# MariusDoe/fractal-ray-marching

Hardware: AMD Instinct MI355X
Metric: Gray-march-steps/sec + frames/sec, 4K Mandelbulb 12-iter/256-step, 1 & 8 GPU (higher is better)
Workload: dtype f32

## Files before the change

### fractal-ray-marching_amd/csrc/frm_render_kernels.h

```cpp
#pragma once
#include "frm_internal.h"
#include "frm_srgb_table.h"

namespace frm {

__device__ __forceinline__ unsigned long long wave_sum(unsigned long long v) {
#pragma unroll
  for (int off = 32; off >= 1; off >>= 1) v += __shfl_xor(v, off, 64);
  return v;
}

__device__ __forceinline__ uint32_t band_row_to_global(const BandGeometry& g, uint32_t lr) {
  uint32_t b = lr / g.band_rows;
  return (g.first_band + b * g.band_stride) * g.band_rows + (lr - b * g.band_rows);
}

template <uint32_t FAM, bool ITERS>
__global__ __launch_bounds__(256) void render_simple(KernelArgs a) {
  __shared__ float table[256];
  table[threadIdx.x] = kSrgbThresholds[threadIdx.x];
  __syncthreads();

  const uint32_t wave = threadIdx.x >> 6, lane = threadIdx.x & 63u;
  const uint32_t x = blockIdx.x * 16u + (wave & 1u) * 8u + (lane & 7u);
  const uint32_t lr = blockIdx.y * 16u + (wave >> 1) * 8u + (lane >> 3);
  const uint32_t width = a.f.width;

  uint32_t n_pix = 0;
  PixelCount pc = {0u, 0u, 0u, 0u, {0u, 0u}};
  if (x < width && lr < a.g.local_rows) {
    const uint32_t y = band_row_to_global(a.g, lr);
    if (y < a.f.height) {
      n_pix = 1;
      v3 color = shade_pixel<FAM, ITERS>(a.f, a.s, x, y, pc);
      a.out[(size_t)lr * width + x] = pack_rgba(color, table);
    }
  }

  unsigned long long v[7] = {n_pix, pc.hit, pc.primary, pc.shadow, pc.normal, pc.de.bodies, pc.de.bailouts};
#pragma unroll
  for (int k = 0; k < 7; ++k) {
    unsigned long long s = wave_sum(v[k]);
    if (lane == 0 && s) atomicAdd(&a.counters[k], s);
  }
}

constexpr uint32_t kIdle = 0xFFFFFFFFu;
constexpr uint32_t kChunk = 64u;


enum Phase : uint32_t { kPrimary = 0, kTap0 = 1, kTap3 = 4, kShadow = 5 };

__device__ __forceinline__ uint32_t uniform(uint32_t v) { return __builtin_amdgcn_readfirstlane(v); }
__device__ __forceinline__ uint32_t queue_part() {
  const uint32_t xcc = __builtin_amdgcn_s_getreg((3 << 11) | 20) & (kXcds - 1u);
  constexpr uint32_t per = kQueueParts / kXcds;
  return xcc * per + (per > 1u ? (blockIdx.x / kXcds) % per : 0u);
}
__device__ __forceinline__ uint64_t count(bool c) { return (uint64_t)__popcll(ballot(c)); }

__device__ __forceinline__ uint8_t cost_key(uint32_t bodies) {
  return (uint8_t)min(255.0f, 16.0f * __log2f((float)bodies + 1.0f));
}

__device__ __forceinline__ uint32_t sys_load(const uint32_t* p) {
  return __hip_atomic_load(p, __ATOMIC_RELAXED, __HIP_MEMORY_SCOPE_SYSTEM);
}
__device__ __forceinline__ void sys_store(uint32_t* p, uint32_t v) {
  __hip_atomic_store(p, v, __ATOMIC_RELAXED, __HIP_MEMORY_SCOPE_SYSTEM);
}
template <class T>
__device__ __forceinline__ T dev_poll(T* p) {
  return __hip_atomic_fetch_add(p, (T)0, __ATOMIC_RELAXED, __HIP_MEMORY_SCOPE_AGENT);
}
template <class T>
__device__ __forceinline__ T dev_load(const T* p) {
  return __hip_atomic_load(p, __ATOMIC_RELAXED, __HIP_MEMORY_SCOPE_AGENT);
}
template <class T>
__device__ __forceinline__ void dev_store(T* p, T v) {
  __hip_atomic_store(p, v, __ATOMIC_RELAXED, __HIP_MEMORY_SCOPE_AGENT);
}
__device__ __forceinline__ void ring_wait_mem() { asm volatile("s_waitcnt vmcnt(0)" ::: "memory"); }
__device__ __forceinline__ uint64_t realtime() { return __builtin_amdgcn_s_memrealtime(); }
constexpr uint64_t kRingWatchdogTicks = 200000000ull;
constexpr unsigned long long kEpochMask = 0xFFFFFFFF00000000ull;
__device__ __forceinline__ unsigned long long epoch_of(uint32_t seq) { return (unsigned long long)seq << 32; }
#ifdef FRM_RING_TRACE
#define RING_TRACE_MIN(r, seq, k) atomicMin(&(r).dev->trace[(seq) & 63u][k], (unsigned long long)realtime())
#define RING_TRACE_MAX(r, seq, k) atomicMax(&(r).dev->trace[(seq) & 63u][k], (unsigned long long)realtime())
#define RING_GRID_TRACE(r, k) atomicMin(&(r).dev->grid_trace[(r).grid_id & 63u][k], (unsigned long long)realtime())
#else
#define RING_TRACE_MIN(r, seq, k)
#define RING_TRACE_MAX(r, seq, k)
#define RING_GRID_TRACE(r, k)
#endif
__device__ __forceinline__ RingFrameCtl& ring_ctl(const RingArgs& r, uint32_t seq) {
  return r.dev->set[(seq - 1u) & (2u * r.slots - 1u)];
}
struct RingLds {
  RingHost* host;
  RingDev* dev;
  uint32_t* order;
  uint32_t slots, grid_id, rec_stride, npix;
};
__device__ __forceinline__ uint32_t rl_u32(const volatile uint32_t& v) { return uniform(v); }
template <class T>
__device__ __forceinline__ T* rl_ptr(T* const volatile& v) {
  const uint64_t x = reinterpret_cast<uint64_t>(v);
  return reinterpret_cast<T*>((uint64_t)uniform((uint32_t)x) | ((uint64_t)uniform((uint32_t)(x >> 32)) << 32));
}
__device__ __forceinline__ RingArgs ring_view(const volatile RingLds* rl) {
  RingArgs r;
  r.host = rl_ptr(rl->host);
  r.dev = rl_ptr(rl->dev);
  r.order = rl_ptr(rl->order);
  r.slots = rl_u32(rl->slots);
  r.grid_id = rl_u32(rl->grid_id);
  r.first_seq = 0;
  r.service_waves = 0;
  r.out = nullptr;
  r.keys = nullptr;
  return r;
}

__device__ __forceinline__ uint32_t epoch_add(unsigned long long* w, uint32_t seq, uint32_t v) {
  unsigned long long old = 0;
  if ((threadIdx.x & 63u) == 0) old = atomicAdd(w, (unsigned long long)v);
  old = __shfl(old, 0, 64);
  return (old & kEpochMask) == epoch_of(seq) ? (uint32_t)old : 0xFFFFFFFFu;
}
__device__ __forceinline__ uint32_t epoch_claim(unsigned long long* w, uint32_t seq, uint32_t n) {
  const uint32_t t = epoch_add(w, seq, 1u);
  return t < n ? t : 0xFFFFFFFFu;
}

struct RingView {
  uint32_t limit;
  bool closed;
};
__device__ __forceinline__ void ring_refresh(const RingArgs& r, RingView& v) {
  if (v.closed) return;
  uint32_t lim = 0, closed = 0;
  if ((threadIdx.x & 63u) == 0) {
    closed = dev_poll(&r.dev->grid.limit_valid);
    if (closed) {
      lim = dev_poll(&r.dev->grid.limit);
    } else {
      const uint32_t posted = sys_load(&r.host->posted);
      const uint32_t stop = sys_load(&r.host->grid_stop[r.grid_id % kRingGridIds][0]);
      lim = min(posted, stop - 1u);
#ifdef FRM_RING_TRACE
      if (lim >= 1u) RING_TRACE_MIN(r, lim, 0);
#endif
    }
  }
  v.closed = uniform(__shfl(closed, 0, 64)) != 0;
  v.limit = uniform(__shfl(lim, 0, 64));
}
__device__ __forceinline__ void ring_close(const RingArgs& r, RingView& v) {
  uint32_t lim = 0, ok = 1;
  if ((threadIdx.x & 63u) == 0) {
    if (atomicCAS(&r.dev->grid.closed, 0u, 1u) == 0u) {
      sys_store(&r.host->closed, r.grid_id);
      RING_GRID_TRACE(r, 1);
      ring_wait_mem();
      const uint32_t posted = sys_load(&r.host->posted);
      const uint32_t stop = sys_load(&r.host->grid_stop[r.grid_id % kRingGridIds][0]);
      lim = min(posted, stop - 1u);
      atomicExch(&r.dev->grid.limit, lim);
      atomicExch(&r.dev->base, lim + 1u);
      ring_wait_mem();
      atomicExch(&r.dev->grid.limit_valid, 1u);
    } else {
      const uint64_t t0 = realtime();
      while (!dev_poll(&r.dev->grid.limit_valid)) {
        if (realtime() - t0 > 1000000ull) { ok = 0; break; }
        __builtin_amdgcn_s_sleep(2);
      }
      lim = dev_poll(&r.dev->grid.limit);
    }
  }
  v.closed = true;
  v.limit = uniform(__shfl(ok ? lim : 0u, 0, 64));
}

struct RingCam {
  float row[3][4];
  v3 origin;
  float power;
  uint32_t* host_img;
};
__device__ __forceinline__ void ring_camera_lds(const RingArgs& r, uint32_t slot, float* lds) {
  const uint32_t* w = reinterpret_cast<const uint32_t*>(&r.host->frames[slot]);
  const uint32_t lane = threadIdx.x & 63u;
  if (lane < 16u) lds[lane] = __uint_as_float(sys_load(w + lane));
  __syncthreads();
}
__device__ __forceinline__ RingCam ring_camera(const RingArgs& r, uint32_t slot) {
  const uint32_t* w = reinterpret_cast<const uint32_t*>(&r.host->frames[slot]);
  const uint32_t lane = threadIdx.x & 63u;
  const uint32_t mine = lane < 20u ? sys_load(w + lane) : 0u;
  RingCam c;
#pragma unroll
  for (int i = 0; i < 12; ++i) c.row[i / 4][i % 4] = __uint_as_float(uniform(__shfl(mine, i, 64)));
  c.origin = mk(__uint_as_float(uniform(__shfl(mine, 12, 64))), __uint_as_float(uniform(__shfl(mine, 13, 64))),
                __uint_as_float(uniform(__shfl(mine, 14, 64))));
  c.power = __uint_as_float(uniform(__shfl(mine, 15, 64)));
  const uint64_t lo = uniform(__shfl(mine, 18, 64)), hi = uniform(__shfl(mine, 19, 64));
  c.host_img = reinterpret_cast<uint32_t*>(lo | (hi << 32));
  return c;
}
// ... 233 lines not shown
    const uint32_t pos = atomicAdd(&cnt[dev_load(&keys[idx])], 1u);
    if (pos < npix) dev_store(&order[pos], idx);
  }
}

__device__ __forceinline__ void ring_finish(const KernelArgs& a, uint32_t seq, uint32_t s) {
  const uint32_t lane = threadIdx.x & 63u;
  const uint32_t next_seq = seq + a.ring.slots;
  RingFrameCtl& c = ring_ctl(a.ring, next_seq);
  const unsigned long long next = epoch_of(next_seq);
  if (lane <= kQueueParts) dev_store(&c.queue[lane * (kQueuePartWords / 2u)], next);
  if (lane == 16u) dev_store(&c.pix_done[0], next);
  if (lane == 17u) dev_store(&c.shade_next[0], next);
  if (lane == 18u) dev_store(&c.shade_done[0], next);
  if (lane == 19u) dev_store(&c.rank_next[0], next);
  if (lane == 20u) dev_store(&c.rank_done[0], next);
#pragma unroll
  for (uint32_t k = 0; k < kRankWords / 64u; ++k) dev_store(&c.hist[k * 64u + lane], 0u);
  __builtin_amdgcn_fence(__ATOMIC_RELEASE, "");
  if (lane == 0) {
    RING_TRACE_MIN(a.ring, seq, 5);
    atomicExch(&a.ring.dev->done_seq[s][0], seq);
    sys_store(&a.ring.host->done[s][0], seq);
  }
}

__device__ __forceinline__ void ring_idle() {
#pragma unroll
  for (int i = 0; i < 4; ++i) __builtin_amdgcn_s_sleep(127);
}

template <uint32_t FAM>
__device__ __noinline__ void ring_service(const KernelArgs& a, uint32_t* cnt) {
  const RingArgs& R = a.ring;
  const uint32_t lane = threadIdx.x & 63u;
  const float* table = kSrgbThresholds;
  const uint32_t npix = a.npix;
  const uint32_t ntask = (npix + kRingTaskPixels - 1u) / kRingTaskPixels;
  uint32_t seq0 = 0;
  if (lane == 0) seq0 = max(R.first_seq, dev_poll(&R.dev->base));
  seq0 = uniform(__shfl(seq0, 0, 64));
  RingView rv = {0u, false};
  uint64_t last_progress = realtime();
  unsigned long long last_pd = 0;
  for (;;) {
    if (seq0 > rv.limit) ring_refresh(R, rv);
    for (;;) {
      if (seq0 > rv.limit) break;
      uint32_t d = 0;
      if (lane == 0) d = dev_poll(&R.dev->done_seq[(seq0 - 1u) & (R.slots - 1u)][0]);
      if (uniform(__shfl(d, 0, 64)) < seq0) break;
      ++seq0;
    }
    if (seq0 > rv.limit) {
      if (rv.closed) return;
      if (realtime() - last_progress > kRingWatchdogTicks) return;
      ring_idle();
      continue;
    }
    bool worked = false;
    for (uint32_t g = seq0; g <= rv.limit && g < seq0 + R.slots && !worked; ++g) {
      const uint32_t s = (g - 1u) & (R.slots - 1u);
      RingFrameCtl& c = ring_ctl(R, g);
      unsigned long long pd = 0, sd = 0;
      if (lane == 0) {
        pd = dev_poll(&c.pix_done[0]);
        sd = dev_poll(&c.shade_done[0]);
      }
      pd = __shfl(pd, 0, 64);
      sd = __shfl(sd, 0, 64);
      if (g == seq0 && pd != last_pd) {
        last_pd = pd;
        last_progress = realtime();
      }
      if (pd != (epoch_of(g) | npix)) continue;
      if (sd == (epoch_of(g) | ntask)) {
        const uint32_t t = epoch_claim(&c.rank_next[0], g, ntask);
        if (t == kIdle) continue;
        ring_rank_task(a, g, s, t, cnt);
        ring_wait_mem();
        if (epoch_add(&c.rank_done[0], g, 1u) == ntask - 1u) ring_finish(a, g, s);
        worked = true;
      } else {
        const uint32_t t = epoch_claim(&c.shade_next[0], g, ntask);
        if (t == kIdle) continue;
        const RingCam cam = ring_camera(R, s);
        ring_shade_task<FAM>(a, cam, g, s, t, table, cnt);
        if (cam.host_img)
          __builtin_amdgcn_fence(__ATOMIC_RELEASE, "");
        else
          ring_wait_mem();
        if (epoch_add(&c.shade_done[0], g, 1u) == ntask - 1u && lane == 0) RING_TRACE_MIN(R, g, 4);
        worked = true;
      }
    }
    if (worked) {
      last_progress = realtime();
    } else {
      if (realtime() - last_progress > kRingWatchdogTicks) return;
      ring_idle();
    }
  }
}

#ifdef FRM_STAMPS
constexpr uint32_t kWaveDebugSlots = 16384u;
__device__ unsigned long long g_wave_debug[16u * kWaveDebugSlots];
#endif

template <uint32_t FAM, bool ITERS, bool MULTI = false, bool ANIM = false, bool RES = false>
#ifndef FRM_MARCH_WAVES_PER_SIMD
#define FRM_MARCH_WAVES_PER_SIMD 1
#endif
#ifndef FRM_RING_WAVES_PER_SIMD
#define FRM_RING_WAVES_PER_SIMD FRM_MARCH_WAVES_PER_SIMD
#endif
__global__ __launch_bounds__(kMarchBlock, RES ? FRM_RING_WAVES_PER_SIMD : FRM_MARCH_WAVES_PER_SIMD) void march_persistent(
    KernelArgs a) {
  __shared__ float4 chunk_rays[kMarchWaves][kChunk];
  static_assert(!RES || (!MULTI && kMarchWaves == 1u), "ring grids: one-wave workgroups, one frame per chunk");
  __shared__ float cam_lds[RES ? kRingSlots : 1][16];
  __shared__ uint32_t rw[RES ? (uint32_t)kRwWords : 1u];
  __shared__ RingLds ring_lds[RES ? 1 : 0 + 1];
  if constexpr (RES) {
    if (blockIdx.x < a.ring.service_waves) {
      ring_service<FAM>(*(const KernelArgs*)__builtin_amdgcn_kernarg_segment_ptr(),
                        reinterpret_cast<uint32_t*>(&chunk_rays[0][0]));
      return;
    }
  }

  const FrameUniforms& f = a.f;
  const SceneUniforms& su = a.s;
  constexpr bool kMb = is_mandelbulb(FAM);
  constexpr bool kHw = FAM == kMandelbulbHw;
  const uint32_t wave = threadIdx.x >> 6, lane = threadIdx.x & 63u;
  const uint64_t lane_bit = 1ull << lane;
  constexpr bool multi = MULTI;
  const uint32_t total = multi ? a.batch * ((a.npix + kChunk - 1u) / kChunk) * kChunk : a.npix;
  uint32_t chunk_frame = 0;
  const uint32_t n_iter = iterations<ITERS>(su.n);
  static_assert(!ANIM || ((MULTI || RES) && is_mandelbulb(FAM)), "per-lane powers: multi-frame or ring Mandelbulb launches");
  float lane_power = su.mb_power;
  ShadeGeom* __restrict__ geom = a.geom;
  ShadeTail* __restrict__ tails = a.tails;

  uint32_t slots_used = kChunk;
  bool exhausted = false;
  const uint32_t nchunks = (total + kChunk - 1u) / kChunk;
  uint32_t part = queue_part();
  uint64_t drained = 0;
  const uint32_t nhead = nchunks / kQueueHeadDiv;
  uint64_t n_pix = 0, n_hit = 0, n_prim = 0, n_shadow = 0, n_body = 0, n_bail = 0;
#ifdef FRM_COUNT_EXACT
  uint64_t n_dbg_total = 0, n_dbg_exact = 0;
#endif
  uint32_t r_slot = 0;
  if constexpr (RES) {
    uint32_t b = 0;
    if (lane == 0) {
      RING_GRID_TRACE(a.ring, 0);
      b = max(a.ring.first_seq, dev_poll(&a.ring.dev->base));
      ring_lds->host = a.ring.host;
      ring_lds->dev = a.ring.dev;
      ring_lds->order = a.ring.order;
      ring_lds->slots = a.ring.slots;
      ring_lds->grid_id = a.ring.grid_id;
      ring_lds->rec_stride = a.rec_stride;
      ring_lds->npix = a.npix;
    }
    __syncthreads();
    if (lane < (uint32_t)kRwWords) rw[lane] = 0u;
    rw_set(rw, kRwLo, uniform(__shfl(b, 0, 64)));
  }

  uint32_t pix = kIdle;
  uint32_t phase = kPrimary;
  bool done = false;
  v3 o = mk(0.f, 0.f, 0.f), d = o, nsum = o, q = o, z = o;
  float t = 0.f, closeness = 0.f, dr = 1.f, mag = 0.f, de = 0.f;
  uint32_t it = 0, psteps = 0, body = 0;
  uint32_t pix_cost = 0;
#ifdef FRM_STAMPS
  uint64_t stamp_service = 0, n_service = 0, n_loop = 0, real_exhaust = 0;
  uint64_t stamp_consume = 0, stamp_refill = 0, n_fetch = 0;
  uint64_t stamp_sub[4] = {0, 0, 0, 0};
  const uint64_t stamp_begin = __builtin_amdgcn_s_memtime();
  const uint64_t stamp_real0 = __builtin_amdgcn_s_memrealtime();
#define FRM_SUB_BEGIN() const uint64_t sub0 = __builtin_amdgcn_s_memtime()
#define FRM_SUB_END(k) stamp_sub[k] += __builtin_amdgcn_s_memtime() - sub0
#else
#define FRM_SUB_BEGIN()
#define FRM_SUB_END(k)
#endif

  for (;;) {
    if constexpr (kMb) {
      const uint64_t live = ballot(pix != kIdle);
      uint64_t pending = live & ~ballot(done);
      const uint64_t waitable = exhausted ? live : ~0ull;
      for (;;) {
        if (pending == 0 || (uint32_t)__popcll(waitable & ~pending) >= a.service_min) break;
        if constexpr (!RES) n_body += (uint64_t)__popcll(pending);
#ifdef FRM_STAMPS
        n_loop++;
#endif
        if (lane_in(pending)) {
#if defined(FRM_COUNT_EXACT) && defined(__HIP_DEVICE_COMPILE__)
          n_dbg_total++;
          if (ballot(!mb_tame(z, mag)) != 0) n_dbg_exact++;
#endif
          if constexpr (ANIM)
            mb_step<kHw>(lane_power, lane_power - 1.0f, q, mag, z, dr);
          else
            mb_step<kHw>(su, q, mag, z, dr);
          body++;
          if (body <= n_iter) mag = mb_length<kHw>(z);
        }
        pending &= ~(ballot(body > n_iter) | ballot(mag > su.mb_bailout));
      }
      done = !lane_in(pending);
    }

#ifdef FRM_STAMPS
    const uint64_t stamp0 = __builtin_amdgcn_s_memtime();
#endif
    const bool cons = pix != kIdle && done;
    bool ev_bail = false;
    bool plain_log = true;
    if constexpr (kMb && !kHw)
      plain_log = ballot(cons && !__builtin_amdgcn_classf(mag, 0x100 )) == 0;
    if (cons) {
      done = false;
      if constexpr (kMb) {
        FRM_SUB_BEGIN();
#if defined(__HIP_DEVICE_COMPILE__)
        if constexpr (kHw)
          de = mb_distance_hw(mag, dr);
        else
          de = plain_log ? mb_distance_posnormal(mag, dr) : mb_distance(mag, dr);
#else
        (void)plain_log;
        de = mb_distance(mag, dr);
#endif
        pix_cost += body;
        ev_bail = body <= n_iter;
        FRM_SUB_END(0);
      }
    }
    const bool ev_prim = cons && phase == kPrimary, ev_shadow = cons && phase == kShadow;
    const bool tap = cons && !ev_prim && !ev_shadow;
    const bool hit = de <= kMinDistance;
    const bool ev_hit = ev_prim && hit;
    const float cl = min_(closeness, de / t);
    closeness = ev_shadow ? cl : closeness;
    const bool step = (ev_prim || ev_shadow) && !hit;
    const float t_next = t + de;
    const uint32_t it_next = it + 1u;
    const bool more = it_next < f.max_steps && t_next < kMaxTotalDistance;
    t = step ? t_next : t;
    it = step ? it_next : it;
    psteps = ev_hit ? it : psteps;
    const bool fin = (step && !more) || (ev_shadow && hit);
    const bool sun_miss = ev_shadow && step && !more;
    bool need_point = ev_hit || (step && more) || tap;
    const uint32_t k = phase - kTap0;
    const float dx = (k == 0u || k == 3u) ? de : -de, dy = (k >= 2u) ? de : -de,
                dz = (k == 1u || k == 3u) ? de : -de;
    const float sx = (k == 0u) ? dx : nsum.x + dx, sy = (k == 0u) ? dy : nsum.y + dy,
                sz = (k == 0u) ? dz : nsum.z + dz;
    nsum = mk(tap ? sx : nsum.x, tap ? sy : nsum.y, tap ? sz : nsum.z);
    phase = ev_hit ? kTap0 : (tap ? phase + 1u : phase);
    if (tap && k == kTap3 - kTap0) {
      FRM_SUB_BEGIN();
#if defined(__HIP_DEVICE_COMPILE__)
      const v3 n = normalize_wave(nsum);
#else
      const v3 n = normalize(nsum);
#endif
      const v3 hp = ray_at(o, t, d);
      if constexpr (RES) {
        coherent_store(&geom[pix], make_float4(t, n.x, n.y, n.z));
      } else {
        *reinterpret_cast<float4*>(&geom[pix]) = make_float4(t, n.x, n.y, n.z);
      }
      o = shadow_origin(hp, n);
      d = to_sun();
      t = 0.f;
      it = 0;
      closeness = kInfinity;
      FRM_SUB_END(2);
    }
    if (fin) {
      FRM_SUB_BEGIN();
      const uint32_t flags = ev_shadow ? (kRecHit | (sun_miss ? kRecSunMiss : 0u)) : 0u;
      const uint32_t ck = cost_key(pix_cost);
      const uint2 tail = make_uint2(__float_as_uint(closeness), psteps | flags | (ck << kRecKeyShift));
      if constexpr (RES)
        coherent_store(&tails[pix], tail);
      else
        *reinterpret_cast<uint2*>(&tails[pix]) = tail;
      if constexpr (RES)
        atomicAdd(&rw[kRwPend + ring_slot_of(pix, rl_u32(ring_lds->rec_stride))], 1u);
      pix = kIdle;
      FRM_SUB_END(3);
    }
    if constexpr (RES) {
      const uint32_t gone = rw_get(rw, kRwGone);
      if (gone) ring_settle(ring_lds, rw, gone, pix);
    }
#ifdef FRM_STAMPS
    const uint64_t stamp1 = __builtin_amdgcn_s_memtime();
    stamp_consume += stamp1 - stamp0;
#endif
    const uint64_t want = ballot(pix == kIdle);
    if (want != 0 && !exhausted) {
      if (slots_used == kChunk) {
        uint32_t base = kIdle;
        if constexpr (RES) {
          base = ring_claim(ring_lds, rw, cam_lds, nchunks, nhead, pix, &r_slot);
        } else {
        if (!(drained >> kQueueParts)) {
          uint32_t j = 0;
          if (lane == 0) j = atomicAdd(a.queue + kQueueParts * kQueuePartWords, 1u);
          j = uniform(__shfl(j, 0, 64));
          if (j < nhead)
            base = j * kChunk;
          else
            drained |= 1ull << kQueueParts;
        }
        while (base == kIdle) {
          uint32_t j = 0;
          if (lane == 0) j = atomicAdd(a.queue + part * kQueuePartWords, 1u);
          j = uniform(__shfl(j, 0, 64));
          const uint32_t c = nhead + j * kQueueParts + part;
          if (c < nchunks) {
            base = c * kChunk;
            break;
          }
          drained |= 1ull << part;
          if ((drained & ((1ull << kQueueParts) - 1ull)) == (1ull << kQueueParts) - 1ull) break;
          do part = (part + 1u) % kQueueParts;
          while ((drained >> part) & 1u);
        }
        }
#ifdef FRM_STAMPS
        n_fetch++;
#endif
        if (base == kIdle) {
          exhausted = true;
#ifdef FRM_STAMPS
          real_exhaust = __builtin_amdgcn_s_memrealtime();
          if (lane == 0) atomicMin(a.debug + 2, (unsigned long long)real_exhaust);
#endif
        } else {
          uint32_t p = kIdle;
          v3 ray = mk(0.f, 0.f, 0.f);
          uint32_t pos0 = base, lim = total;
          [[maybe_unused]] float row[3][4];
          if constexpr (RES) {
            uint32_t mine = __float_as_uint(cam_lds[r_slot][lane & 15u]);
            asm volatile("" : "+v"(mine));
#pragma unroll
            for (int i = 0; i < 12; ++i) row[i / 4][i % 4] = __uint_as_float(__builtin_amdgcn_readlane(mine, i));
          }
          if constexpr (multi) {
            const uint32_t c = base / kChunk;
            chunk_frame = uniform(c % a.batch);
            pos0 = (c / a.batch) * kChunk;
            lim = a.npix;
          }
          if (pos0 + lane < lim) {
            const uint32_t lp =
                RES ? dev_load(&rl_ptr(((const volatile RingLds*)ring_lds)->order)[r_slot * a.rec_stride + pos0 + lane])
                    : a.pixel_order[pos0 + lane];
            const uint32_t lr = lp / f.width, x = lp - lr * f.width, y = band_row_to_global(a.g, lr);
            if constexpr (RES)
              ray = camera_ray_rows(f, row, x, y);
            else if constexpr (multi)
              ray = camera_ray_rows(f, a.cams[chunk_frame].row, x, y);
            else
              ray = camera_ray(f, x, y);
            p = (RES ? r_slot * a.rec_stride : chunk_frame * a.rec_stride) + lp;
          }
          if constexpr (!RES) n_pix += count(p != kIdle);
          chunk_rays[wave][lane] = make_float4(ray.x, ray.y, ray.z, __uint_as_float(p));
          __builtin_amdgcn_wave_barrier();
          slots_used = 0;
        }
      }
      if (slots_used < kChunk) {
        const uint32_t slot = slots_used + __popcll(want & (lane_bit - 1ull));
        [[maybe_unused]] float cam_o[4];
        if constexpr (RES) {
          uint32_t mine = __float_as_uint(cam_lds[r_slot][12u + (lane & 3u)]);
          asm volatile("" : "+v"(mine));
#pragma unroll
          for (int i = 0; i < 4; ++i) cam_o[i] = __uint_as_float(__builtin_amdgcn_readlane(mine, i));
        }
        if ((want & lane_bit) && slot < kChunk) {
          const float4 r = chunk_rays[wave][slot];
          pix = __float_as_uint(r.w);
          if (pix != kIdle) {
            const uint32_t fy = RES ? 0u : a.first_info[chunk_frame];
            const bool first_skip = (fy & kFirstSkip) != 0u;
            pix_cost = first_skip ? (fy & kFirstCostMask) : 0u;
            d = mk(r.x, r.y, r.z);
            if constexpr (RES)
              o = mk(cam_o[0], cam_o[1], cam_o[2]);
            else
              o = multi ? a.cams[chunk_frame].origin : f.origin;
            if constexpr (RES && ANIM)
              lane_power = cam_o[3];
            else if constexpr (ANIM)
              lane_power = a.mb_powers[chunk_frame];
            t = first_skip ? a.first_t[chunk_frame] : 0.f;
            it = first_skip ? 1u : 0u;
            phase = kPrimary;
            need_point = true;
          }
        }
        slots_used = min(kChunk, slots_used + (uint32_t)__popcll(want));
      }
    }

#ifdef FRM_STAMPS
    stamp_refill += __builtin_amdgcn_s_memtime() - stamp1;
#endif
    if (need_point) {
      const v3 r = ray_at(o, t, d);
      const uint32_t kq = phase - kTap0;
      const bool is_tap = kq <= kTap3 - kTap0;
      const float e = kMinDistance;
      const float ex = (kq == 0u || kq == 3u) ? e : -e, ey = (kq >= 2u) ? e : -e, ez = (kq == 1u || kq == 3u) ? e : -e;
      q = mk(is_tap ? r.x + ex : r.x, is_tap ? r.y + ey : r.y, is_tap ? r.z + ez : r.z);
      if constexpr (kMb) {
        z = q;
        dr = 1.f;
        body = 0;
        mag = mb_length<kHw>(q);
        done = mag > su.mb_bailout;
      } else {
        DeCount unused = {0u, 0u};
        de = scene_de<FAM, ITERS>(su, q, unused);
        done = true;
        pix_cost++;
      }
    }

    if constexpr (!RES) {
      n_prim += count(ev_prim);
      n_hit += count(ev_hit);
      n_shadow += count(ev_shadow);
      n_bail += count(ev_bail);
    }
#ifdef FRM_STAMPS
    stamp_service += __builtin_amdgcn_s_memtime() - stamp0;
    n_service++;
#endif

    if (exhausted && ballot(pix != kIdle) == 0) break;
  }
  if constexpr (RES) {
#pragma unroll
    for (uint32_t sl = 0; sl < kRingSlots; ++sl)
      if (sl < a.ring.slots) ring_flush(ring_lds, rw, sl);
  }

#ifdef FRM_STAMPS
  if (lane == 0) {
    atomicAdd(&a.counters[7], (unsigned long long)stamp_service);
    atomicAdd(a.debug, (unsigned long long)(__builtin_amdgcn_s_memtime() - stamp_begin));
    atomicAdd(a.debug + 1, (unsigned long long)n_service);
    atomicMin(a.debug + 3, (unsigned long long)stamp_real0);
    atomicMax(a.debug + 4, (unsigned long long)__builtin_amdgcn_s_memrealtime());
  }
  {
    const uint32_t w = blockIdx.x * kMarchWaves + wave;
    uint32_t hw = 0;
    asm volatile("s_getreg_b32 %0, hwreg(HW_REG_HW_ID)" : "=s"(hw));
    if (lane == 0 && w < kWaveDebugSlots) {
      unsigned long long* r = g_wave_debug + 16u * w;
      r[8] = stamp_consume;
      r[9] = stamp_refill;
      r[10] = n_fetch;
      for (int k = 0; k < 4; ++k) r[11 + k] = stamp_sub[k];
      r[0] = n_loop;
      r[1] = n_body;
      r[2] = n_service;
      r[3] = stamp_service;
      r[4] = __builtin_amdgcn_s_memtime() - stamp_begin;
      r[5] = stamp_real0;
      r[6] = real_exhaust;
      r[7] = ((unsigned long long)hw << 32) | (uint32_t)(__builtin_amdgcn_s_memrealtime() - stamp_real0);
    }
  }
#endif
  if (lane == 0 && !RES) {
#ifdef FRM_COUNT_EXACT
    atomicAdd(&a.counters[7], (unsigned long long)((n_dbg_total << 32) | n_dbg_exact));
#endif
    if (blockIdx.x == 0 && wave == 0) {
      n_prim += a.first_counts[0];
      n_body += a.first_counts[1];
      n_bail += a.first_counts[2];
    }
    unsigned long long v[7] = {n_pix, n_hit, n_prim, n_shadow, 4ull * n_hit, n_body, n_bail};
#pragma unroll
    for (int k = 0; k < 7; ++k)
      if (v[k]) atomicAdd(&a.counters[k], v[k]);
  }
}

__device__ __forceinline__ uint32_t block_exclusive_scan256(uint32_t v, uint32_t* wave_tot) {
  const uint32_t lane = threadIdx.x & 63u, wave = threadIdx.x >> 6;
  uint32_t inc = v;
#pragma unroll
  for (int off = 1; off < 64; off <<= 1) {
    const uint32_t u = __shfl_up(inc, off, 64);
    if (lane >= (uint32_t)off) inc += u;
  }
  if (lane == 63u) wave_tot[wave] = inc;
  __syncthreads();
  uint32_t before = 0;
  for (uint32_t w = 0; w < wave; ++w) before += wave_tot[w];
  return before + inc - v;
}

template <uint32_t FAM>
__device__ __forceinline__ void shade_record(const KernelArgs& a, uint2 r1, uint32_t rec, uint32_t fr, uint32_t idx,
                                             uint32_t x, uint32_t y, const float* table) {
  uint32_t word = 255u << 24;
  if (r1.y & kRecHit) {
    const float4 r0 = *reinterpret_cast<const float4*>(&a.geom[rec]);
    const bool multi = a.batch > 1u;
    const v3 dir = multi ? camera_ray_rows(a.f, a.cams[fr].row, x, y) : camera_ray(a.f, x, y);
    const v3 hp = ray_at(multi ? a.cams[fr].origin : a.f.origin, r0.x, dir);
    const v3 n = mk(r0.y, r0.z, r0.w);
    float spec;
    v3 color = shade_hit_pre(a.f, scene_color<FAM>(hp), dir, n, r1.y & kRecStepsMask, &spec);
    color = shade_hit_post(color, spec, (r1.y & kRecSunMiss) ? -kInfinity : 0.0f, __uint_as_float(r1.x));
    word = pack_rgba(color, table);
  }
  a.out[(size_t)fr * a.out_stride + idx] = word;
}

template <uint32_t FAM>
__global__ __launch_bounds__(256) void shade_pass(KernelArgs a) {
  __shared__ float table[256];
  __shared__ uint32_t s_count[256];
  const uint32_t t = threadIdx.x;
  const uint32_t fr = blockIdx.y;
  const bool hist = a.key_hist != nullptr && fr + 1u == a.batch;
  table[t] = kSrgbThresholds[t];
  if (hist) s_count[t] = 0u;
  __syncthreads();
  const uint32_t width = a.f.width, local = a.g.local_rows * width;
  for (uint32_t j = 0; j < kShadeBlockPixels / 256u; ++j) {
    const uint32_t idx = (blockIdx.x * (kShadeBlockPixels / 256u) + j) * 256u + t;
    if (idx >= local) break;
    const uint32_t lr = idx / width, x = idx - lr * width;
    const uint32_t y = band_row_to_global(a.g, lr);
    if (y >= a.f.height) break;
    const uint32_t rec = fr * a.rec_stride + idx;
    const uint2 r1 = *reinterpret_cast<const uint2*>(&a.tails[rec]);
    const uint32_t key = r1.y >> kRecKeyShift;
    if (a.pixel_key && fr + 1u == a.batch) a.pixel_key[idx] = (uint8_t)key;
    if (hist) atomicAdd(&s_count[key], 1u);
    shade_record<FAM>(a, r1, rec, fr, idx, x, y, table);
  }
  if (!hist) return;
  __syncthreads();
  if (const uint32_t c = s_count[t]) atomicAdd(a.key_hist + t, c);
  if (blockIdx.x == 0) {
    a.key_hist_next[t] = 0u;
    a.key_hist_next[256u + t] = 0u;
    for (uint32_t w = t; w < kQueueDebugWord; w += 256u) a.queue[w] = 0u;
  }
}

__global__ __launch_bounds__(256) void rank_pass(const uint8_t* __restrict__ keys, uint32_t npix,
                                                 uint32_t* __restrict__ hist, uint32_t* __restrict__ order) {
  constexpr uint32_t kPer = kShadeBlockPixels / 256u;
  __shared__ uint32_t s_base[256], s_count[256], s_res[256], s_wave[4];
  const uint32_t t = threadIdx.x;
  s_count[t] = 0u;
  __syncthreads();
  uint32_t key[kPer], rank[kPer];
#pragma unroll
  for (uint32_t j = 0; j < kPer; ++j) {
    const uint32_t idx = (blockIdx.x * kPer + j) * 256u + t;
    key[j] = idx < npix ? keys[idx] : 0u;
    rank[j] = idx < npix ? atomicAdd(&s_count[key[j]], 1u) : 0u;
  }
  const uint32_t k_desc = 255u - t;
  s_base[k_desc] = block_exclusive_scan256(hist[k_desc], s_wave);
  const uint32_t c = s_count[t];
  s_res[t] = c ? atomicAdd(hist + 256u + t, c) : 0u;
  __syncthreads();
#pragma unroll
  for (uint32_t j = 0; j < kPer; ++j) {
    const uint32_t idx = (blockIdx.x * kPer + j) * 256u + t;
    const uint32_t pos = s_base[key[j]] + s_res[key[j]] + rank[j];
    if (idx < npix && pos < npix) order[pos] = idx;
  }
}

}
```

### fractal-ray-marching_amd/csrc/frm_scene.h

```cpp
#pragma once
#include "frm_math.h"
#include "frm_fast.h"

#if defined(__clang__)
#define FRM_ASSUME(c) __builtin_assume(c)
#else
#define FRM_ASSUME(c) \
  do {                \
    if (!(c)) __builtin_unreachable(); \
  } while (0)
#endif

namespace frm {

template <bool ITERS>
FRM_HD uint32_t iterations(uint32_t n) {
  if (!ITERS) return 0u;
  FRM_ASSUME(n >= 1u);
  return n;
}

enum Family : uint32_t {
  kMenger = 0,
  kSierpinski = 1,
// ... 63 lines not shown
}
FRM_HD float tetrahedron(const SceneUniforms& u, v3 p) {
  float h0 = dot(p - u.tet[0].anchor, u.tet[0].normal);
  float h1 = dot(p - u.tet[1].anchor, u.tet[1].normal);
  float h2 = dot(p - u.tet[2].anchor, u.tet[2].normal);
  float h3 = dot(p - u.tet[3].anchor, u.tet[3].normal);
  return max_(max_(max_(h0, h1), h2), h3);
}

template <bool ITERS, bool FAST>
FRM_HD float menger_folds(const SceneUniforms& u, v3 p, float d) {
  const uint32_t n = iterations<ITERS>(u.n);
  float scale = 1.0f;
  float rcp = FAST ? u.menger_rcp[0] : 0.0f;
  for (uint32_t i = 0; i < n; ++i) {
    const float rcp_next = FAST ? u.menger_rcp[i + 1u < kMengerFastMax ? i + 1u : kMengerFastMax - 1u] : 0.0f;
    v3 r = p * scale;
    v3 c = mk(fract_(r.x + 0.5f) - 0.5f, fract_(r.y + 0.5f) - 0.5f, fract_(r.z + 0.5f) - 0.5f);
    v3 a = abs3(c);
    float cx = max_(a.y, a.z), cy = max_(a.z, a.x), cz = max_(a.x, a.y);
    float ci = min_(min_(cx, cy), cz) - u.menger_cross;
#if defined(__HIP_DEVICE_COMPILE__)
    const float q = FAST ? div_by_rcp(-ci, scale, rcp) : (-ci) / scale;
    if constexpr (FAST)
      d = max_quiet(d, q);
    else
      d = max_(d, q);
#else
    (void)rcp;
    const float q = (-ci) / scale;
    d = max_(d, q);
#endif
    scale = scale * u.menger_factor;
    rcp = rcp_next;
  }
  return d;
}
template <bool ITERS>
FRM_HD float de_menger(const SceneUniforms& u, v3 p) {
  v3 q = mk(fabsf(p.x) - 0.5f, fabsf(p.y) - 0.5f, fabsf(p.z) - 0.5f);
  float d = length(max3s(q, 0.0f)) + min_(max_(max_(q.x, q.y), q.z), 0.0f);
#if defined(__HIP_DEVICE_COMPILE__)
  if (u.menger_fast) return menger_folds<ITERS, true>(u, p, d);
#endif
  return menger_folds<ITERS, false>(u, p, d);
}

template <bool ITERS>
FRM_HD float de_sierpinski(const SceneUniforms& u, v3 p) {
  const uint32_t n = iterations<ITERS>(u.n);
  v3 q = mk(p.x, p.y + u.sp_yoff, p.z);
  v3 top = mk(0.0f, u.sp_top_y, 0.0f);
  for (uint32_t j = 0; j < n; ++j) {
    const uint32_t i = n - 1u - j;
    float dist = (float)(int32_t)(1u << (i & 31u));
    q = mirror(q, fma3(dist, u.sp_top[0], top), u.sp_normal[0]);
    q = mirror(q, fma3(dist, u.sp_top[1], top), u.sp_normal[1]);
    q = mirror(q, fma3(dist, u.sp_top[2], top), u.sp_normal[2]);
  }
  return tetrahedron(u, q);
}

template <bool ITERS>
FRM_HD float de_koch(const SceneUniforms& u, v3 p) {
  const uint32_t n = iterations<ITERS>(u.n);
  v3 q = p * 2.0f;
  for (uint32_t i = 0; i < n; ++i) {
    q = q * 1.5f;
    q = mk(q.y, q.x, q.z);
    q = mirror0(q, u.koch_n1);
    q = mirror0(q, u.koch_n2);
    q.z = q.z - u.koch_offset;
  }
  q.y = fabsf(q.y);
  return tetrahedron(u, q) / u.koch_scale;
}

FRM_HD void mb_body(float P, float Pm1, v3 c, float r, v3& z, float& dr) {
  float theta = acos_(z.z / r);
  float phi = atan2_(z.y, z.x);
  float l2 = log2_(r);
  const float pm1 = exp2_(Pm1 * l2);
  dr = fma_(pm1 * P, dr, 1.0f);
  float er = pm1 * r;
  float st, ct, sp, cp;
  sincos_(theta * P, &st, &ct);
  sincos_(phi * P, &sp, &cp);
  z = mk(fma_(er, st * cp, c.x), fma_(er, sp * st, c.y), fma_(er, ct, c.z));
}
#if defined(__HIP_DEVICE_COMPILE__)
__device__ __forceinline__ float hw_sqrt(float x) { return __builtin_amdgcn_sqrtf(x); }
__device__ __forceinline__ float hw_div(float a, float b) { return a * __builtin_amdgcn_rcpf(b); }
__device__ __forceinline__ void hw_sincos(float x, float* s, float* c) {
  const float rev = x * 0.15915494309189535f;
  *s = __builtin_amdgcn_sinf(rev);
  *c = __builtin_amdgcn_cosf(rev);
}
__device__ __forceinline__ float hw_acos(float t) {
  float a = fabsf(t);
  bool big = a > 0.5f;
  float zb = 0.5f * (1.0f - a);
  float z = big ? zb : a * a;
  float w = big ? hw_sqrt(zb) : a;
  float p = fma_(fma_(fma_(fma_(4.2163199048e-2f, z, 2.4181311049e-2f), z, 4.5470025998e-2f), z,
                      7.4953002686e-2f), z, 1.6666752422e-1f);
  float s = fma_(w * z, p, w);
  float rb = (t > 0.0f) ? 2.0f * s : kPi - 2.0f * s;
  return big ? rb : kHalfPi - copysignf(s, t);
}
__device__ __forceinline__ float hw_atan2(float y, float x) {
  float ax = fabsf(x), ay = fabsf(y);
  float mx = fmaxf(ax, ay), mn = fminf(ax, ay);
  float a = mx == 0.0f ? 0.0f : hw_div(mn, mx);
  float s = a * a;
  float q = fma_(fma_(fma_(fma_(fma_(fma_(fma_(0.002974590389872539f, s, -0.016581183968493302f), s,
                                      0.04355353931255974f), s, -0.07580578130128461f), s,
                          0.10678940285181907f), s, -0.14214209135918496f), s,
                0.1999413720560495f), s, -0.3333316696611865f);
  float r = fma_(a * s, q, a);
  r = (ay > ax) ? kHalfPi - r : r;
  r = (x < 0.0f) ? kPi - r : r;
  return copysignf(r, y);
}
__device__ __forceinline__ void mb_body_hw(float P, float Pm1, v3 c, float r, v3& z, float& dr) {
  float theta = hw_acos(hw_div(z.z, r));
  float phi = hw_atan2(z.y, z.x);
  float l2 = __builtin_amdgcn_logf(r);
  dr = fma_(__builtin_amdgcn_exp2f(Pm1 * l2) * P, dr, 1.0f);
  float er = __builtin_amdgcn_exp2f(P * l2);
  float st, ct, sp, cp;
  hw_sincos(theta * P, &st, &ct);
  hw_sincos(phi * P, &sp, &cp);
  z = mk(fma_(er, st * cp, c.x), fma_(er, sp * st, c.y), fma_(er, ct, c.z));
}
__device__ __forceinline__ float mb_distance_hw(float r, float dr) {
  return hw_div((0.5f * (__builtin_amdgcn_logf(r) * 0.6931471805599453f)) * r, dr);
}
#endif

FRM_HD float mb_distance(float r, float dr) { return ((0.5f * log_(r)) * r) / dr; }
FRM_HD float mb_distance_posfinite(float r, float dr) { return ((0.5f * log_posfinite_(r)) * r) / dr; }
#if defined(__HIP_DEVICE_COMPILE__)
__device__ __forceinline__ float mb_distance_posnormal(float r, float dr) {
  return ((0.5f * log_posnormal(r)) * r) / dr;
}
#endif

#if defined(__HIPCC__)
__device__ __forceinline__ uint64_t ballot(bool b) {
#if defined(__HIP_DEVICE_COMPILE__)
  return __builtin_amdgcn_ballot_w64(b);
#else
  return b;
#endif
}
__device__ __forceinline__ bool lane_in(uint64_t mask) {
#if defined(__HIP_DEVICE_COMPILE__) && __has_builtin(__builtin_amdgcn_inverse_ballot_w64)
  return __builtin_amdgcn_inverse_ballot_w64(mask);
#else
  return (mask >> (threadIdx.x & 63u)) & 1u;
#endif
}
#endif

#if defined(__HIP_DEVICE_COMPILE__)
__device__ __forceinline__ bool mb_tame(v3 z, float r) {
  float m;
  asm("v_min3_f32 %0, |%1|, |%2|, |%3|" : "=v"(m) : "v"(z.x), "v"(z.y), "v"(z.z));
  return (r >= 0x1p-13f) & (m >= 0x1p-60f);
}

__device__ __forceinline__ void mb_body_tame(float P, float Pm1, v3 c, float r, v3& z, float& dr) {
  float theta = acos_dev(div_tame_nz(z.z, r));
  float phi = atan2_tame(z.y, z.x);
  float l2 = log2_tame(r);
  const float pm1 = exp2_tame(Pm1 * l2);
  dr = fma_(pm1 * P, dr, 1.0f);
  float er = pm1 * r;
  float st, ct, sp, cp;
  uint32_t tt, tp;
  sincos_unsigned(theta * P, &st, &ct, &tt);
  sincos_unsigned(phi * P, &sp, &cp, &tp);
  const float er_xy = __uint_as_float(__float_as_uint(er) ^ ((tt + tp) << 31));
  const float er_z = __uint_as_float(__float_as_uint(er) ^ (tt << 31));
  z = mk(fma_(er_xy, st * cp, c.x), fma_(er_xy, sp * st, c.y), fma_(er_z, ct, c.z));
}

__device__ __forceinline__ float length_rsq(v3 a) { return sqrt_rsq(dot(a, a)); }
__device__ __forceinline__ bool length_wide(v3 a) {
  constexpr uint32_t kLo = 0x0f800000u, kHi = 0x7e800000u;
  return __float_as_uint(dot(a, a)) - kLo > kHi - kLo;
}

__device__ __forceinline__ bool normalize_wide(v3 a) {
  float m;
  asm("v_min3_f32 %0, |%1|, |%2|, |%3|" : "=v"(m) : "v"(a.x), "v"(a.y), "v"(a.z));
  return length_wide(a) | !(m >= 0x1p-62f);
}
__device__ __forceinline__ v3 normalize_rsq(v3 a) {
  const float l = length_rsq(a);
  const float y = rcp_rn(l);
  return mk(div_by_rcp_fix(a.x, l, y), div_by_rcp_fix(a.y, l, y), div_by_rcp_fix(a.z, l, y));
}
__device__ __forceinline__ v3 normalize_wave(v3 a) {
  return ballot(normalize_wide(a)) == 0 ? normalize_rsq(a) : normalize(a);
}

#endif


template <bool HW = false>
FRM_HD void mb_step(float P, float Pm1, v3 c, float r, v3& z, float& dr) {
#if defined(__HIP_DEVICE_COMPILE__)
  if constexpr (HW) {
    mb_body_hw(P, Pm1, c, r, z, dr);
    return;
  }
  if (ballot(!mb_tame(z, r)) == 0) {
    mb_body_tame(P, Pm1, c, r, z, dr);
    return;
  }
#endif
  mb_body(P, Pm1, c, r, z, dr);
}
template <bool HW = false>
FRM_HD void mb_step(const SceneUniforms& u, v3 c, float r, v3& z, float& dr) {
  mb_step<HW>(u.mb_power, u.mb_power_m1, c, r, z, dr);
}
template <bool HW = false>
FRM_HD float mb_length(v3 z) {
#if defined(__HIP_DEVICE_COMPILE__)
  if constexpr (HW) return hw_sqrt(dot(z, z));
  if (ballot(length_wide(z)) == 0) return length_rsq(z);
#endif
  return length(z);
}

template <bool ITERS, bool HW = false>
FRM_HD float de_mandelbulb(const SceneUniforms& u, v3 p, DeCount& cnt) {
  const uint32_t n = iterations<ITERS>(u.n);
  v3 z = p;
  float dr = 1.0f;
  float r = 0.0f;
  for (uint32_t i = 0;; ++i) {
    r = mb_length<HW>(z);
    if (r > u.mb_bailout) {
      cnt.bailouts++;
      break;
    }
    mb_step<HW>(u, p, r, z, dr);
    cnt.bodies++;
    if (i == n) break;
  }
#if defined(__HIP_DEVICE_COMPILE__)
  if constexpr (HW) return mb_distance_hw(r, dr);
#endif
  return mb_distance(r, dr);
}

FRM_HD float de_sphere(v3 p) { return length(p) - 0.5f; }

template <uint32_t FAM, bool ITERS>
FRM_HD float scene_de(const SceneUniforms& u, v3 p, DeCount& cnt) {
  if constexpr (FAM == kMenger) return de_menger<ITERS>(u, p);
  else if constexpr (FAM == kSierpinski) return de_sierpinski<ITERS>(u, p);
  else if constexpr (FAM == kKoch) return de_koch<ITERS>(u, p);
  else if constexpr (FAM == kMandelbulb) return de_mandelbulb<ITERS>(u, p, cnt);
  else if constexpr (FAM == kMandelbulbHw) return de_mandelbulb<ITERS, true>(u, p, cnt);
  else return de_sphere(p);
}

template <uint32_t FAM>
FRM_HD v3 scene_color(v3 p) {
  if constexpr (FAM == kSierpinski) return colorize(p * 1.5f);
  else return colorize(p);
}

FRM_HD float screen_x(uint32_t x, uint32_t w) { return (float)(2u * x + 1u) / (float)w - 1.0f; }
FRM_HD float screen_y(uint32_t y, uint32_t h) { return 1.0f - (float)(2u * y + 1u) / (float)h; }

FRM_HD v3 camera_ray_rows(const FrameUniforms& f, const float (&row)[3][4], uint32_t x, uint32_t y) {
  float sx = screen_x(x, f.width), sy = screen_y(y, f.height);
  v3 d = normalize(mk(sx * f.aspect_x, sy * f.aspect_y, kCameraDirectionZ));
  v3 o;
  o.x = fma_(0.0f, row[0][3], fma_(d.z, row[0][2], fma_(d.y, row[0][1], d.x * row[0][0])));
  o.y = fma_(0.0f, row[1][3], fma_(d.z, row[1][2], fma_(d.y, row[1][1], d.x * row[1][0])));
  o.z = fma_(0.0f, row[2][3], fma_(d.z, row[2][2], fma_(d.y, row[2][1], d.x * row[2][0])));
  return o;
}
FRM_HD v3 camera_ray(const FrameUniforms& f, uint32_t x, uint32_t y) { return camera_ray_rows(f, f.row, x, y); }

struct FrameCamera {
  float row[3][4];
  v3 origin;
};

FRM_HD v3 to_sun() { return mk(kToSunX, kToSunY, kToSunZ); }

FRM_HD v3 normal_from_taps(float d0, float d1, float d2, float d3) {
  v3 s = mk(((d0 - d1) - d2) + d3, ((-d0 - d1) + d2) + d3, ((-d0 + d1) - d2) + d3);
  return normalize(s);
}
FRM_HD v3 normal_tap_pos(v3 p, int k) {
  const float e = kMinDistance;
  switch (k) {
    case 0: return mk(p.x + e, p.y + -e, p.z + -e);
// ... 112 lines not shown
```

Before: 56.06.

## Compute march-loop event predicates as wave-wide masks with lean all-primary pass

Replaces per-lane boolean event logic in the persistent march loop with 64-bit wave masks (ballots combined with scalar bit ops), so counters come from popcounts and the done state is kept as a mask. It adds an inline-asm class_mask helper and a 'lean' path that skips the tap/shadow/normal bookkeeping when every live lane is on a primary ray. By default the lean path is enabled only for non-Mandelbulb families. The aim is to move VALU predicate work onto scalar mask operations and drop redundant ballots, at the cost of more code-path complexity and a possible increase in register pressure.

Result: slower. 54.19 (-3.3%).

```diff
diff --git a/fractal-ray-marching_amd/csrc/frm_render_kernels.h b/fractal-ray-marching_amd/csrc/frm_render_kernels.h
--- a/fractal-ray-marching_amd/csrc/frm_render_kernels.h
+++ b/fractal-ray-marching_amd/csrc/frm_render_kernels.h
@@ -57,7 +57,7 @@
   constexpr uint32_t per = kQueueParts / kXcds;
   return xcc * per + (per > 1u ? (blockIdx.x / kXcds) % per : 0u);
 }
-__device__ __forceinline__ uint64_t count(bool c) { return (uint64_t)__popcll(ballot(c)); }
+__device__ __forceinline__ uint64_t count(uint64_t lanes) { return (uint64_t)__popcll(lanes); }
 
 __device__ __forceinline__ uint8_t cost_key(uint32_t bodies) {
   return (uint8_t)min(255.0f, 16.0f * __log2f((float)bodies + 1.0f));
@@ -597,7 +597,10 @@
   uint64_t drained = 0;
   const uint32_t nhead = nchunks / kQueueHeadDiv;
   uint64_t n_pix = 0, n_hit = 0, n_prim = 0, n_shadow = 0, n_body = 0, n_bail = 0;
-#ifdef FRM_COUNT_EXACT
+#if defined(FRM_COUNT_EXACT) && defined(FRM_COUNT_PASSES)
+#error "FRM_COUNT_EXACT and FRM_COUNT_PASSES both report through counters[7]"
+#endif
+#if defined(FRM_COUNT_EXACT) || defined(FRM_COUNT_PASSES)
   uint64_t n_dbg_total = 0, n_dbg_exact = 0;
 #endif
   uint32_t r_slot = 0;
@@ -621,7 +624,14 @@
 
   uint32_t pix = kIdle;
   uint32_t phase = kPrimary;
-  bool done = false;
+  constexpr bool kMasks = !RES;
+#ifdef FRM_LEAN_PASS_ALL
+  constexpr bool kLeanPass = kMasks;
+#else
+  constexpr bool kLeanPass = kMasks && !kMb;
+#endif
+  [[maybe_unused]] uint64_t done = 0;
+  [[maybe_unused]] bool done_flag = false;
   v3 o = mk(0.f, 0.f, 0.f), d = o, nsum = o, q = o, z = o;
   float t = 0.f, closeness = 0.f, dr = 1.f, mag = 0.f, de = 0.f;
   uint32_t it = 0, psteps = 0, body = 0;
@@ -640,9 +650,9 @@
 #endif
 
   for (;;) {
+    const uint64_t live = ballot(pix != kIdle);
     if constexpr (kMb) {
-      const uint64_t live = ballot(pix != kIdle);
-      uint64_t pending = live & ~ballot(done);
+      uint64_t pending = live & ~(kMasks ? done : ballot(done_flag));
       const uint64_t waitable = exhausted ? live : ~0ull;
       for (;;) {
         if (pending == 0 || (uint32_t)__popcll(waitable & ~pending) >= a.service_min) break;
@@ -664,19 +674,28 @@
         }
         pending &= ~(ballot(body > n_iter) | ballot(mag > su.mb_bailout));
       }
-      done = !lane_in(pending);
+      done = ~pending;
+      done_flag = !lane_in(pending);
     }
 
 #ifdef FRM_STAMPS
     const uint64_t stamp0 = __builtin_amdgcn_s_memtime();
 #endif
-    const bool cons = pix != kIdle && done;
-    bool ev_bail = false;
+    bool cons, ev_hit, ev_shadow, tap, fin, sun_miss, lean = false;
+    [[maybe_unused]] bool need_point = false;
+    [[maybe_unused]] uint64_t cons_m = 0, need_m = 0;
     bool plain_log = true;
-    if constexpr (kMb && !kHw)
-      plain_log = ballot(cons && !__builtin_amdgcn_classf(mag, 0x100 )) == 0;
+    if constexpr (kMasks) {
+      cons_m = kMb ? live & done : live;
+      cons = lane_in(cons_m);
+      if constexpr (kMb && !kHw) plain_log = (cons_m & ~class_mask<0x100 >(mag)) == 0;
+    } else {
+      cons = pix != kIdle && done_flag;
+      if constexpr (kMb && !kHw)
+        plain_log = ballot(cons && !__builtin_amdgcn_classf(mag, 0x100 )) == 0;
+    }
     if (cons) {
-      done = false;
+      done_flag = false;
       if constexpr (kMb) {
         FRM_SUB_BEGIN();
 #if defined(__HIP_DEVICE_COMPILE__)
@@ -689,52 +708,92 @@
         de = mb_distance(mag, dr);
 #endif
         pix_cost += body;
-        ev_bail = body <= n_iter;
         FRM_SUB_END(0);
       }
     }
-    const bool ev_prim = cons && phase == kPrimary, ev_shadow = cons && phase == kShadow;
-    const bool tap = cons && !ev_prim && !ev_shadow;
-    const bool hit = de <= kMinDistance;
-    const bool ev_hit = ev_prim && hit;
-    const float cl = min_(closeness, de / t);
-    closeness = ev_shadow ? cl : closeness;
-    const bool step = (ev_prim || ev_shadow) && !hit;
     const float t_next = t + de;
     const uint32_t it_next = it + 1u;
-    const bool more = it_next < f.max_steps && t_next < kMaxTotalDistance;
-    t = step ? t_next : t;
-    it = step ? it_next : it;
+    if constexpr (kMasks) {
+      const uint64_t on_primary = ballot(phase == kPrimary);
+      const bool all_primary = (live & ~on_primary) == 0;
+#ifdef FRM_COUNT_PASSES
+      n_dbg_total++;
+      if (all_primary) n_dbg_exact++;
+#endif
+      if constexpr (kLeanPass) lean = all_primary;
+      const uint64_t prim_m = cons_m & on_primary;
+      const uint64_t hit_m = ballot(de <= kMinDistance);
+      const uint64_t ev_hit_m = prim_m & hit_m;
+      uint64_t shadow_m = 0, tap_m = 0;
+      if (!lean) {
+        shadow_m = cons_m & ballot(phase == kShadow);
+        tap_m = cons_m & ~(prim_m | shadow_m);
+        const float cl = min_(closeness, de / t);
+        closeness = lane_in(shadow_m) ? cl : closeness;
+      }
+      n_prim += count(prim_m);
+      n_hit += count(ev_hit_m);
+      n_shadow += count(shadow_m);
+      if constexpr (kMb) n_bail += count(cons_m & ballot(body <= n_iter));
+      const uint64_t step_m = (prim_m | shadow_m) & ~hit_m;
+      const uint64_t more_m = ballot(it_next < f.max_steps) & ballot(t_next < kMaxTotalDistance);
+      const uint64_t end_m = step_m & ~more_m;
+      need_m = ev_hit_m | (step_m & more_m) | tap_m;
+      ev_hit = lane_in(ev_hit_m);
+      ev_shadow = lane_in(shadow_m);
+      tap = lane_in(tap_m);
+      fin = lane_in(end_m | (shadow_m & hit_m));
+      sun_miss = lane_in(shadow_m & end_m);
+      const bool step = lane_in(step_m);
+      t = step ? t_next : t;
+      it = step ? it_next : it;
+    } else {
+      const bool ev_prim = cons && phase == kPrimary;
+      ev_shadow = cons && phase == kShadow;
+      tap = cons && !ev_prim && !ev_shadow;
+      const bool hit = de <= kMinDistance;
+      ev_hit = ev_prim && hit;
+      const float cl = min_(closeness, de / t);
+      closeness = ev_shadow ? cl : closeness;
+      const bool step = (ev_prim || ev_shadow) && !hit;
+      const bool more = it_next < f.max_steps && t_next < kMaxTotalDistance;
+      t = step ? t_next : t;
+      it = step ? it_next : it;
+      fin = (step && !more) || (ev_shadow && hit);
+      sun_miss = ev_shadow && step && !more;
+      need_point = ev_hit || (step && more) || tap;
+    }
     psteps = ev_hit ? it : psteps;
-    const bool fin = (step && !more) || (ev_shadow && hit);
-    const bool sun_miss = ev_shadow && step && !more;
-    bool need_point = ev_hit || (step && more) || tap;
-    const uint32_t k = phase - kTap0;
-    const float dx = (k == 0u || k == 3u) ? de : -de, dy = (k >= 2u) ? de : -de,
-                dz = (k == 1u || k == 3u) ? de : -de;
-    const float sx = (k == 0u) ? dx : nsum.x + dx, sy = (k == 0u) ? dy : nsum.y + dy,
-                sz = (k == 0u) ? dz : nsum.z + dz;
-    nsum = mk(tap ? sx : nsum.x, tap ? sy : nsum.y, tap ? sz : nsum.z);
-    phase = ev_hit ? kTap0 : (tap ? phase + 1u : phase);
-    if (tap && k == kTap3 - kTap0) {
-      FRM_SUB_BEGIN();
+    if (lean) {
+      phase = ev_hit ? kTap0 : phase;
+    } else {
+      const uint32_t k = phase - kTap0;
+      const float dx = (k == 0u || k == 3u) ? de : -de, dy = (k >= 2u) ? de : -de,
+                  dz = (k == 1u || k == 3u) ? de : -de;
+      const float sx = (k == 0u) ? dx : nsum.x + dx, sy = (k == 0u) ? dy : nsum.y + dy,
+                  sz = (k == 0u) ? dz : nsum.z + dz;
+      nsum = mk(tap ? sx : nsum.x, tap ? sy : nsum.y, tap ? sz : nsum.z);
+      phase = ev_hit ? kTap0 : (tap ? phase + 1u : phase);
+      if (tap && k == kTap3 - kTap0) {
+        FRM_SUB_BEGIN();
 #if defined(__HIP_DEVICE_COMPILE__)
-      const v3 n = normalize_wave(nsum);
+        const v3 n = normalize_wave(nsum);
 #else
-      const v3 n = normalize(nsum);
-#endif
-      const v3 hp = ray_at(o, t, d);
-      if constexpr (RES) {
-        coherent_store(&geom[pix], make_float4(t, n.x, n.y, n.z));
-      } else {
-        *reinterpret_cast<float4*>(&geom[pix]) = make_float4(t, n.x, n.y, n.z);
-      }
-      o = shadow_origin(hp, n);
-      d = to_sun();
-      t = 0.f;
-      it = 0;
-      closeness = kInfinity;
-      FRM_SUB_END(2);
+        const v3 n = normalize(nsum);
+#endif
+        const v3 hp = ray_at(o, t, d);
+        if constexpr (RES) {
+          coherent_store(&geom[pix], make_float4(t, n.x, n.y, n.z));
+        } else {
+          *reinterpret_cast<float4*>(&geom[pix]) = make_float4(t, n.x, n.y, n.z);
+        }
+        o = shadow_origin(hp, n);
+        d = to_sun();
+        t = 0.f;
+        it = 0;
+        closeness = kInfinity;
+        FRM_SUB_END(2);
+      }
     }
     if (fin) {
       FRM_SUB_BEGIN();
@@ -828,7 +887,7 @@
               ray = camera_ray(f, x, y);
             p = (RES ? r_slot * a.rec_stride : chunk_frame * a.rec_stride) + lp;
           }
-          if constexpr (!RES) n_pix += count(p != kIdle);
+          if constexpr (!RES) n_pix += count(ballot(p != kIdle));
           chunk_rays[wave][lane] = make_float4(ray.x, ray.y, ray.z, __uint_as_float(p));
           __builtin_amdgcn_wave_barrier();
           slots_used = 0;
@@ -872,39 +931,40 @@
 #ifdef FRM_STAMPS
     stamp_refill += __builtin_amdgcn_s_memtime() - stamp1;
 #endif
-    if (need_point) {
+    const uint64_t live_next = ballot(pix != kIdle);
+    if constexpr (kMasks) need_m |= want & live_next;
+    if (kMasks ? lane_in(need_m) : need_point) {
       const v3 r = ray_at(o, t, d);
-      const uint32_t kq = phase - kTap0;
-      const bool is_tap = kq <= kTap3 - kTap0;
       const float e = kMinDistance;
-      const float ex = (kq == 0u || kq == 3u) ? e : -e, ey = (kq >= 2u) ? e : -e, ez = (kq == 1u || kq == 3u) ? e : -e;
-      q = mk(is_tap ? r.x + ex : r.x, is_tap ? r.y + ey : r.y, is_tap ? r.z + ez : r.z);
+      if (lean) {
+        q = mk(ev_hit ? r.x + e : r.x, ev_hit ? r.y + -e : r.y, ev_hit ? r.z + -e : r.z);
+      } else {
+        const uint32_t kq = phase - kTap0;
+        const bool is_tap = kq <= kTap3 - kTap0;
+        const float ex = (kq == 0u || kq == 3u) ? e : -e, ey = (kq >= 2u) ? e : -e, ez = (kq == 1u || kq == 3u) ? e : -e;
+        q = mk(is_tap ? r.x + ex : r.x, is_tap ? r.y + ey : r.y, is_tap ? r.z + ez : r.z);
+      }
       if constexpr (kMb) {
         z = q;
         dr = 1.f;
         body = 0;
         mag = mb_length<kHw>(q);
-        done = mag > su.mb_bailout;
+        done_flag = mag > su.mb_bailout;
       } else {
         DeCount unused = {0u, 0u};
         de = scene_de<FAM, ITERS>(su, q, unused);
-        done = true;
+        done_flag = true;
         pix_cost++;
       }
     }
-
-    if constexpr (!RES) {
-      n_prim += count(ev_prim);
-      n_hit += count(ev_hit);
-      n_shadow += count(ev_shadow);
-      n_bail += count(ev_bail);
-    }
+    if constexpr (kMb && kMasks) done = need_m & ballot(mag > su.mb_bailout);
+
 #ifdef FRM_STAMPS
     stamp_service += __builtin_amdgcn_s_memtime() - stamp0;
     n_service++;
 #endif
 
-    if (exhausted && ballot(pix != kIdle) == 0) break;
+    if (exhausted && live_next == 0) break;
   }
   if constexpr (RES) {
 #pragma unroll
@@ -942,7 +1002,7 @@
   }
 #endif
   if (lane == 0 && !RES) {
-#ifdef FRM_COUNT_EXACT
+#if defined(FRM_COUNT_EXACT) || defined(FRM_COUNT_PASSES)
     atomicAdd(&a.counters[7], (unsigned long long)((n_dbg_total << 32) | n_dbg_exact));
 #endif
     if (blockIdx.x == 0 && wave == 0) {
diff --git a/fractal-ray-marching_amd/csrc/frm_scene.h b/fractal-ray-marching_amd/csrc/frm_scene.h
--- a/fractal-ray-marching_amd/csrc/frm_scene.h
+++ b/fractal-ray-marching_amd/csrc/frm_scene.h
@@ -239,6 +239,16 @@
   return __builtin_amdgcn_ballot_w64(b);
 #else
   return b;
+#endif
+}
+template <uint32_t CLASS>
+__device__ __forceinline__ uint64_t class_mask(float x) {
+#if defined(__HIP_DEVICE_COMPILE__)
+  uint64_t m;
+  asm("v_cmp_class_f32_e64 %0, %1, %2" : "=s"(m) : "v"(x), "s"(CLASS));
+  return m;
+#else
+  return 0;
 #endif
 }
 __device__ __forceinline__ bool lane_in(uint64_t mask) {
```
